# ezorita/seeq

Hardware: AMD Instinct MI355X
Metric: lines/s scanned (20 bp pattern, d=3, 150 bp reads; GB/s in gb_per_s) (higher is better)
Workload: dtype int (u16 automaton state ids; exact-pass columns u32 bit-vectors)

## Files before the change

seeq_amd/csrc/seeq_pair.h:

```cpp
#ifndef SEEQ_PAIR_H_
#define SEEQ_PAIR_H_

#define PAIR_X2(K) \
   asm("v_xor_b32_sdwa %0, %1, %2 dst_sel:DWORD dst_unused:UNUSED_PAD src0_sel:DWORD src1_sel:BYTE_" #K : "=v"(ada) : "v"(sa), "v"(ta)); \
   asm("v_xor_b32_sdwa %0, %1, %2 dst_sel:DWORD dst_unused:UNUSED_PAD src0_sel:DWORD src1_sel:BYTE_" #K : "=v"(adb) : "v"(sb), "v"(tb)); \
   sa = *(stream_lds_cu16 *)(uintptr_t)ada; sb = *(stream_lds_cu16 *)(uintptr_t)adb; \
   __builtin_amdgcn_sched_barrier(0);

__device__ __forceinline__ uint32_t pair_prep(uint32_t w)
{
   const uint32_t u = w & 0x06060606u;
   return u | (u << 10);
}

__device__ __forceinline__ void pair_chk(uint32_t w, uint32_t &bad, uint32_t &nm, bool first_of_two)
{
   const uint32_t idx = (w >> 1) & 0x07070707u;
   bad = __builtin_amdgcn_sad_u8(w, __builtin_amdgcn_perm(0x4EFF0AFFu, 0x47544341u, idx), bad);
   const uint32_t nf = __builtin_amdgcn_perm(0x00000100u, 0u, idx);
   nm = first_of_two ? __builtin_amdgcn_udot4(nf, 0x10204080u, nm << 8, false) : __builtin_amdgcn_udot4(nf, 0x01020408u, nm, false);
}

__device__ __forceinline__ void pair_warm4x2(uint32_t &sa, uint32_t wa, uint32_t &sb, uint32_t wb, uint32_t &seena, uint32_t &seenb)
{
   const uint32_t ta = pair_prep(wa), tb = pair_prep(wb);
   uint32_t ada, adb;
   PAIR_X2(1) asm("v_or_b32 %0, %0, %1" : "+v"(seena) : "v"(sa)); asm("v_or_b32 %0, %0, %1" : "+v"(seenb) : "v"(sb));
   PAIR_X2(3) asm("v_or_b32 %0, %0, %1" : "+v"(seena) : "v"(sa)); asm("v_or_b32 %0, %0, %1" : "+v"(seenb) : "v"(sb));
}

template <bool CHK>
__device__ __forceinline__ void pair_own4x2(uint32_t &sa, uint32_t wa, uint32_t &hma, uint32_t &nma, uint32_t &sb, uint32_t wb, uint32_t &hmb, uint32_t &nmb,
                                            uint32_t &bad, bool first_of_two)
{
   const uint32_t ta = pair_prep(wa), tb = pair_prep(wb);
   uint32_t ada, adb;
   PAIR_X2(1)
   asm volatile("" : "+v"(wa));
   if (CHK) pair_chk(wa, bad, nma, first_of_two);
   asm volatile("" : "+v"(bad), "+v"(nma));
   __builtin_amdgcn_sched_barrier(0);
   hma = __builtin_amdgcn_alignbit(sa, hma, 1); hmb = __builtin_amdgcn_alignbit(sb, hmb, 1);
   asm volatile("" : "+v"(hma), "+v"(hmb));
   PAIR_X2(3)
   asm volatile("" : "+v"(wb));
   if (CHK) pair_chk(wb, bad, nmb, first_of_two);
   asm volatile("" : "+v"(bad), "+v"(nmb));
   __builtin_amdgcn_sched_barrier(0);
   hma = __builtin_amdgcn_alignbit(sa, hma, 1); hmb = __builtin_amdgcn_alignbit(sb, hmb, 1);
   asm volatile("" : "+v"(hma), "+v"(hmb));
}

__device__ __forceinline__ uint32_t pair_word8(const fused_v4u &p, const fused_v4u &q, int k)
{
   return k == 0 ? p.x : k == 1 ? p.y : k == 2 ? p.z : k == 3 ? p.w : k == 4 ? q.x : k == 5 ? q.y : k == 6 ? q.z : q.w;
}

typedef uint32_t pair_u32_unaligned __attribute__((aligned(1)));

__device__ __forceinline__ uint32_t pair_nonbase_mask32(const fused_v4u &a, const fused_v4u &b)
{
   const uint32_t w[8] = {a.x, a.y, a.z, a.w, b.x, b.y, b.z, b.w};
   uint32_t h[2];
#pragma unroll
   for (int g = 0; g < 2; g++) {
      uint32_t acc = 0;
#pragma unroll
      for (int k = 4 * g; k < 4 * g + 4; k += 2) {
         uint32_t f[2];
#pragma unroll
         for (int u = 0; u < 2; u++) {
            const uint32_t x = w[k + u];
            const uint32_t t = x ^ __builtin_amdgcn_perm(0x474E5554u, 0x43FF41FFu, x & 0x07070707u);
            f[u] = (((t & 0x5F5F5F5Fu) + 0x7F7F7F7Fu) | t) & 0x80808080u;
         }
         acc = __builtin_amdgcn_udot4(f[0], 0x10204080u, __builtin_amdgcn_udot4(f[1], 0x01020408u, acc << 8, false), false);
      }
      h[g] = acc;
   }
   return (h[0] << 9) | (h[1] >> 7);
}

__device__ __forceinline__ uint32_t pair_count_before(const uint32_t (&m)[4], const uint32_t (&c)[5], uint32_t b)
{
   const uint32_t r = b >> 5, lz = b & 31u;
   const uint32_t mr = r == 0 ? m[0] : r == 1 ? m[1] : r == 2 ? m[2] : r == 3 ? m[3] : 0u;
   const uint32_t cr = r == 0 ? c[0] : r == 1 ? c[1] : r == 2 ? c[2] : r == 3 ? c[3] : c[4];
   return cr + (lz ? (uint32_t)__popc(mr >> (32u - lz)) : 0u);
}

template <int WU, bool CHK>
__device__ __forceinline__ void pair_walk(const fused_v4u (&v)[8], uint32_t halo, bool halo_nl, uint32_t (&hm)[2], uint32_t (&nmask)[4], uint32_t &tile_bad)
{
   constexpr int NQ = 8, NM = 4;
   uint32_t sa = 0, sb = 0, hma = 0, hmb = 0, seena = 0, seenb = 0, bad = 0, nma = 0, nmb = 0;
#pragma unroll
   for (int k = 8 - WU; k < 8; k++)
      pair_warm4x2(sa, stream_from_prev_lane(pair_word8(v[NQ - 2], v[NQ - 1], k), halo_nl ? 0x0A0A0A0Au : (uint32_t)__builtin_amdgcn_readlane((int)halo, k)),
                        sb, pair_word8(v[NQ / 2 - 2], v[NQ / 2 - 1], k), seena, seenb);
#pragma unroll
   for (int q = 0; q < NQ / 2; q++) {
      pair_own4x2<CHK>(sa, v[q].x, hma, nma, sb, v[q + NQ / 2].x, hmb, nmb, bad, true);
      pair_own4x2<CHK>(sa, v[q].y, hma, nma, sb, v[q + NQ / 2].y, hmb, nmb, bad, false);
      pair_own4x2<CHK>(sa, v[q].z, hma, nma, sb, v[q + NQ / 2].z, hmb, nmb, bad, true);
      pair_own4x2<CHK>(sa, v[q].w, hma, nma, sb, v[q + NQ / 2].w, hmb, nmb, bad, false);
      if (CHK && (q & 1)) { nmask[q >> 1] = nma; nmask[(q >> 1) + NM / 2] = nmb; nma = 0; nmb = 0; }
   }
   tile_bad = bad;
   hm[0] = __builtin_bitreverse32(hma) | ((seena & 1u) << 31);
   hm[1] = __builtin_bitreverse32(hmb) | ((seenb & 1u) << 31);
}

template <int WU, bool FA, bool IG = false, bool LL = false>
__global__ __launch_bounds__(64 * STREAM_NW, 8) void k_pair(FusedArgs a)
{
   static_assert(!(FA && IG), "SQ_IGNORE on FASTA input stays with k_stream");
   static_assert(!(LL && (FA || IG)), "the long-line variant serves plain text under SQ_FAIL / SQ_CONVERT");
   constexpr int NW = STREAM_NW;
   constexpr int CH = 128;
   constexpr int NQ = CH / 16;
   constexpr int NM = CH / 32;
   constexpr uint32_t TB = 64u * CH;
   static_assert(WU >= 4 && WU <= 8, "warm-up is 16 .. 32 bytes");
   extern __shared__ __align__(16) uint8_t dsmem[];
   const int tid = threadIdx.x, lane = tid & 63;
   const int wave = __builtin_amdgcn_readfirstlane(tid >> 6);
   {
      const fused_v4u *src = reinterpret_cast<const fused_v4u *>(a.dfa);
      for (uint32_t i = tid; i < a.dfa_rows; i += 64 * NW) reinterpret_cast<fused_v4u *>(dsmem)[i] = src[i];
   }
   __syncthreads();

   const uint32_t gwave = blockIdx.x * NW + wave, nwaves = gridDim.x * NW;
   if (a.clk_probe != nullptr && blockIdx.x == 0 && tid == 0) { a.clk_probe[0] = __builtin_readcyclecounter(); a.clk_probe[1] = wall_clock64(); }
   uint32_t wv_lines = 0, wv_hitlines = 0, wv_hdrs = 0, slice_pos = 0;
   bool wv_overflow = false;
   uint32_t wv_dirty = 0, wv_lastnl = 0;
   uint32_t dmode = 0;
   uint4 *slice = a.tmp + (size_t)gwave * a.slice_cap;
   const uint64_t lim = a.seg_base + a.seg_len;
   const uint64_t last = a.nbytes - 1;

   fused_v4u v[NQ];
   uint32_t halo = 0;
   uint32_t tile = gwave;
   while (tile < a.ntiles) {
      const uint64_t t0 = a.seg_base + (uint64_t)tile * TB;
      const bool partial = tile + 1 == a.ntiles && (a.seg_len % TB) != 0;
      const uint32_t next = tile + nwaves;
      uint32_t lane_off = (uint32_t)lane * CH;
      asm volatile("" : "+v"(lane_off));
      const uint64_t my = t0 + lane_off;
      {
         if (!partial) {
            const uint8_t *p = a.text + my;
#pragma unroll
            for (int q = 0; q < NQ; q++) v[q] = *reinterpret_cast<const fused_v4u_unaligned *>(p + 16 * q);
            uint32_t lid;
            asm volatile("v_mbcnt_lo_u32_b32 %0, -1, 0\n\tv_mbcnt_hi_u32_b32 %0, -1, %0" : "=v"(lid));
            halo = *reinterpret_cast<const pair_u32_unaligned *>(a.text + (t0 >= 32 ? t0 - 32 : 0) + ((lid & 7u) << 2));
         } else {
#pragma unroll
            for (int q = 0; q < NQ; q++) v[q] = dfa_load16(a.text, my + 16 * q, lim);
            const fused_v4u h0 = dfa_load16(a.text, t0 >= 32 ? t0 - 32 : 0, lim), h1 = dfa_load16(a.text, t0 >= 32 ? t0 - 16 : 0, lim);
            halo = pair_word8(h0, h1, 0);
#pragma unroll
            for (int k = 1; k < 8; k++) halo = (lane & 7) == k ? pair_word8(h0, h1, k) : halo;
         }
      }
      const bool halo_nl = t0 < 32;
      uint32_t hm[2], nmask[NM];
      if (!dmode) {
         uint32_t tile_bad;
         pair_walk<WU, true>(v, halo, halo_nl, hm, nmask, tile_bad);
         const uint64_t badlanes = __ballot(tile_bad != 0);
         dmode = (uint32_t)__builtin_amdgcn_readfirstlane(badlanes != 0 ? 1 : 0);
         if (LL && lane == 0) { a.tile_dirty[tile] = badlanes != 0 ? 1u : 0u; a.tile_dmask[tile] = badlanes; }
      } else {
         uint32_t unused;
         pair_walk<WU, false>(v, halo, halo_nl, hm, nmask, unused);
         if (LL && lane == 0) { a.tile_dirty[tile] = 1u; a.tile_dmask[tile] = ~0ull; }
      }
      if (dmode) {
         wv_dirty |= 1u;
#pragma unroll
         for (int r = 0; r < NM; r++) nmask[r] = stream_nl_mask32(v[2 * r], v[2 * r + 1], false);
      }
      uint32_t valid = CH;
      if (partial) {
         valid = lim > my ? (lim - my < CH ? (uint32_t)(lim - my) : (uint32_t)CH) : 0u;
#pragma unroll
         for (int r = 0; r < NM; r++) {
            const uint32_t lo = 32u * r;
            nmask[r] &= valid <= lo ? 0u : (valid >= lo + 32 ? 0xFFFFFFFFu : ~(0xFFFFFFFFu >> (valid - lo)));
         }
#pragma unroll
         for (int x = 0; x < 2; x++) {
            const uint32_t vx = valid <= 64u * x ? 0u : (valid - 64u * x >= 64u ? 64u : valid - 64u * x);
            const uint32_t np = (vx + 1u) >> 1;
            hm[x] &= np >= 32u ? 0xFFFFFFFFu : ~(0xFFFFFFFFu >> np);
         }
      }
      uint32_t mk[2] = {0u, 0u};
      const uint32_t walk_hm[2] = {hm[0], hm[1]};
      if (IG) {
         uint32_t e_tail = 0;
         if (t0 <= last && last < t0 + TB) { if (a.text[last] != '\n') e_tail = (uint32_t)(last - t0) + 1u; }
         else if (!partial && a.text[t0 + TB] == '\n') e_tail = TB;
         e_tail = (uint32_t)__builtin_amdgcn_readfirstlane((int)e_tail);
         uint32_t vm[NM], sk[NM], dn[NM];
#pragma unroll
         for (int r = 0; r < NM; r++) {
            const uint32_t lo = 32u * r;
            vm[r] = valid <= lo ? 0u : (valid >= lo + 32 ? 0xFFFFFFFFu : ~(0xFFFFFFFFu >> (valid - lo)));
            sk[r] = dmode ? pair_nonbase_mask32(v[2 * r], v[2 * r + 1]) & ~nmask[r] & vm[r] : 0u;
            dn[r] = ~(nmask[r] | sk[r]) & vm[r];
         }
         uint32_t cD[5], cS[5];
         cD[0] = 0; cS[0] = 0;
#pragma unroll
         for (int r = 0; r < NM; r++) { cD[r + 1] = cD[r] + (uint32_t)__popc(dn[r]); cS[r + 1] = cS[r] + (uint32_t)__popc(sk[r]); }
         const uint32_t end_after = (uint32_t)__builtin_amdgcn_update_dpp(0, (int)(nmask[0] >> 31), 0x130, 0xf, 0xf, true);
         uint32_t b_tail = 0;
         if (e_tail && (uint32_t)lane == (e_tail - 1u) / CH) b_tail = e_tail - (uint32_t)lane * CH;
         if (end_after) b_tail = CH;
         uint32_t baseD = 0, baseS = 0, seen_end = 0, firstP = 0, first_pq = 0;
         auto mark = [&](uint32_t pq) { if (pq < 32u) mk[0] |= 0x80000000u >> pq; else mk[1] |= 0x80000000u >> (pq - 32u); };
         auto line_end = [&](uint32_t b, uint32_t Dc, uint32_t Sc) {
            if (b >= 1u) {
               const uint32_t lineD = Dc + baseD, lineS = Sc + baseS;
               if (!seen_end) { firstP = 0x80000000u | (lineS << 14) | lineD; first_pq = (b - 1u) >> 1; }
               else if (lineS != 0u && lineD >= a.ig_thr) mark((b - 1u) >> 1);
            }
            baseD = 0u - Dc; baseS = 0u - Sc; seen_end = 1u;
         };
#pragma unroll
         for (int r = 0; r < NM; r++) {
            uint32_t mm = nmask[r];
            while (mm) {
               const uint32_t lz = (uint32_t)__builtin_clz(mm);
               mm &= ~(0x80000000u >> lz);
               line_end(32u * r + lz, cD[r] + (uint32_t)__popc((dn[r] >> 1) >> (31u - lz)), cS[r] + (uint32_t)__popc((sk[r] >> 1) >> (31u - lz)));
            }
         }
         if (__ballot(b_tail != 0u)) {
            if (b_tail == CH) line_end(CH, cD[4], cS[4]);
            else if (b_tail) line_end(b_tail, pair_count_before(dn, cD, b_tail), pair_count_before(sk, cS, b_tail));
         }
         uint32_t P = (seen_end << 31) | (cD[4] + baseD) | ((cS[4] + baseS) << 14);
#define PAIR_SEG(ctrl, rmask) { const uint32_t y = (uint32_t)__builtin_amdgcn_update_dpp(0, (int)P, ctrl, rmask, 0xf, true); P = (P >> 31) ? P : y + P; }
         PAIR_SEG(0x111, 0xf) PAIR_SEG(0x112, 0xf) PAIR_SEG(0x114, 0xf) PAIR_SEG(0x118, 0xf) PAIR_SEG(0x142, 0xa) PAIR_SEG(0x143, 0xc)
#undef PAIR_SEG
         const uint32_t starts_line = (uint32_t)__builtin_amdgcn_readfirstlane((t0 == 0 || (t0 >= 32 && ((uint32_t)__builtin_amdgcn_readlane((int)halo, 7) >> 24) == 0x0Au)) ? 1 : 0);
         const uint32_t before = stream_from_prev_lane(P, starts_line << 31);
         if ((firstP >> 31) && ((before >> 31) | starts_line)) {
            const uint32_t sum = (firstP & 0x0FFFFFFFu) + (before & 0x0FFFFFFFu);
            if ((sum >> 14) != 0u && (sum & 0x3FFFu) >= a.ig_thr) mark(first_pq);
         }
         {
            const uint32_t tile_valid = (uint32_t)__builtin_amdgcn_readfirstlane((int)(partial ? (uint32_t)(lim - t0) : TB));
            const uint32_t lv = (tile_valid - 1u) >> 7, bb = (tile_valid - 1u) & 127u;
            const uint32_t ng = (bb >> 5) == 0 ? nmask[0] : (bb >> 5) == 1 ? nmask[1] : (bb >> 5) == 2 ? nmask[2] : nmask[3];
            const uint32_t last_is_nl = (uint32_t)__builtin_amdgcn_readlane((int)((ng >> (31u - (bb & 31u))) & 1u), (int)lv);
            const bool buffer_last = t0 <= last && last < t0 + TB;
            if (!buffer_last && e_tail == 0u && !last_is_nl) {
               const uint32_t P63 = (uint32_t)__builtin_amdgcn_readlane((int)P, 63);
               const uint32_t started_here = (P63 >> 31) | starts_line;
               const uint64_t pk = t0 + tile_valid + 4u * (uint32_t)lane;
               uint32_t w = 0x0A0A0A0Au;
               if (pk + 4 <= a.nbytes) w = *reinterpret_cast<const pair_u32_unaligned *>(a.text + pk);
               else for (int i = 3; i >= 0; i--) w = (w << 8) | (pk + (uint64_t)i < a.nbytes ? (uint32_t)a.text[pk + i] : 0x0Au);
               const uint32_t nlf = nl_flags(w);
               const uint64_t nlb = __ballot(nlf != 0u);
               uint32_t qualifies = 1u;
               if (nlb != 0ull && started_here) {
                  const uint32_t F = (uint32_t)__builtin_ctzll(nlb);
                  const uint32_t nbytes_mine = (uint32_t)lane < F ? 4u : (uint32_t)lane == F ? ((uint32_t)__builtin_ctz(nlf) >> 3) : 0u;
                  const uint32_t keepm = nbytes_mine >= 4u ? 0xFFFFFFFFu : (1u << (8u * nbytes_mine)) - 1u;
                  const uint32_t y = (w ^ __builtin_amdgcn_perm(0x474E5554u, 0x43FF41FFu, w & 0x07070707u)) & keepm;
                  const uint32_t cs = (uint32_t)__popc((((y & 0x5F5F5F5Fu) + 0x7F7F7F7Fu) | y) & 0x80808080u);
                  const uint32_t tot = (uint32_t)__builtin_amdgcn_readlane((int)wave_incl_scan_u32((nbytes_mine - cs) | (cs << 16)), 63);
                  const uint32_t lineD = (P63 & 0x3FFFu) + (tot & 0xFFFFu), lineS = ((P63 >> 14) & 0x3FFFu) + (tot >> 16);
                  qualifies = (lineS != 0u && lineD >= a.ig_thr) ? 1u : 0u;
               }
               if (qualifies && (uint32_t)lane == lv) mark(bb >> 1);
            }
         }
         hm[0] |= mk[0]; hm[1] |= mk[1];
      }
      if (t0 <= last && last < t0 + TB) {
         const uint32_t o = (uint32_t)(last - t0);
         if ((uint32_t)lane == o / CH) {
            const uint32_t pos = o % CH;
#pragma unroll
            for (int r = 0; r < NM; r++)
               if ((pos >> 5) == (uint32_t)r) nmask[r] &= ~(0x80000000u >> (pos & 31));
         }
      }
      if (!LL && __ballot(((hm[0] & (hm[0] - 1u)) | (hm[1] & (hm[1] - 1u))) != 0)) {
#pragma unroll
         for (int x = 0; x < 2; x++) {
            const uint32_t n0 = nmask[2 * x], n1 = nmask[2 * x + 1], h = hm[x];
            const uint32_t f = n0 ? (uint32_t)__builtin_clz(n0) : (n1 ? 32u + (uint32_t)__builtin_clz(n1) : 64u);
            const uint32_t l = n1 ? 63u - (uint32_t)__builtin_ctz(n1) : (n0 ? 31u - (uint32_t)__builtin_ctz(n0) : 64u);
            const uint32_t na = f >= 64u ? 32u : (f + 1u) >> 1;
            const uint32_t sc = f >= 64u ? 32u : (l + 1u) >> 1;
            const uint32_t ma = na >= 32u ? 0xFFFFFFFFu : ~(0xFFFFFFFFu >> na);
            const uint32_t mc = sc >= 32u ? 0u : 0xFFFFFFFFu >> sc;
            const uint32_t ha = h & ma, hc = h & mc & ~ma;
            hm[x] = (h & ~ma & ~mc) | (ha ? (0x80000000u >> (uint32_t)__builtin_clz(ha)) | (ha & (0u - ha)) : 0u)
                                    | (hc ? (0x80000000u >> (uint32_t)__builtin_clz(hc)) | (hc & (0u - hc)) : 0u);
         }
      }
      uint32_t lane_nl = 0;
      const uint32_t lane_hits = (uint32_t)__popc(hm[0]) + (uint32_t)__popc(hm[1]);
#pragma unroll
      for (int r = 0; r < NM; r++) lane_nl += (uint32_t)__popc(nmask[r]);
      const uint32_t incl_h = wave_incl_scan_u32(lane_hits), incl_n = wave_incl_scan_u32(lane_nl);
      const uint32_t tot_h = (uint32_t)__builtin_amdgcn_readlane((int)incl_h, 63);
      const uint32_t tot_n = (uint32_t)__builtin_amdgcn_readlane((int)incl_n, 63);
      const uint32_t extra = (uint32_t)__builtin_amdgcn_readfirstlane((a.first_seg && tile == 0) ? 1 : 0);
      uint32_t dmask[NM], lane_hd = 0, excl_d = 0, tot_d = 0, hd_extra = 0;
#pragma unroll
      for (int r = 0; r < NM; r++) dmask[r] = 0;
      if (FA) {
#pragma unroll
         for (int r = 0; r < NM; r++) {
            uint32_t mm = nmask[r];
            while (mm) {
               const uint32_t lz = (uint32_t)__builtin_clz(mm);
               mm &= ~(0x80000000u >> lz);
               const uint64_t nxt = my + 32u * r + lz + 1;
               if (a.text[nxt] == '>') dmask[r] |= 0x80000000u >> lz;
            }
            lane_hd += (uint32_t)__popc(dmask[r]);
         }
         const uint32_t incl_d = wave_incl_scan_u32(lane_hd);
         excl_d = incl_d - lane_hd;
         tot_d = (uint32_t)__builtin_amdgcn_readlane((int)incl_d, 63);
         hd_extra = extra && a.text[0] == '>' ? 1u : 0u;
      }
      uint32_t incl_last = 0;
      if (tot_n && (tot_h || LL)) {
         uint32_t my_last = 0;
#pragma unroll
         for (int r = 0; r < NM; r++)
            if (nmask[r]) my_last = (uint32_t)lane * CH + 32u * r + (31u - (uint32_t)__builtin_ctz(nmask[r])) + 2u;
         incl_last = wave_incl_max_u32(my_last);
         if (LL) wv_lastnl = tile * TB + (uint32_t)__builtin_amdgcn_readlane((int)incl_last, 63) - 1u;
      }
      if (tot_h) {
         if (slice_pos + tot_h <= a.slice_cap) {
            uint32_t before = stream_from_prev_lane(incl_last, 0u);
            if (extra && before == 0) before = 1;
            if (lane_hits) {
               uint32_t ord = incl_h - lane_hits;
               uint32_t nlb = incl_n - lane_nl + extra - 1u - excl_d - hd_extra;
#pragma unroll
               for (int r = 0; r < NM; r++) {
                  uint32_t mm = (r & 1) ? hm[r >> 1] << 16 : hm[r >> 1] & 0xFFFF0000u;
                  const uint32_t mkm = (r & 1) ? mk[r >> 1] << 16 : mk[r >> 1] & 0xFFFF0000u;
                  const uint32_t wkm = (r & 1) ? walk_hm[r >> 1] << 16 : walk_hm[r >> 1] & 0xFFFF0000u;
                  while (mm) {
                     const uint32_t lp = (uint32_t)__builtin_clz(mm);
                     mm &= ~(0x80000000u >> lp);
                     const uint32_t isk = IG ? (((mkm << lp) >> 31) << 30) | ((((mkm & wkm) << lp) >> 31) << 29) : 0u;
                     uint32_t lz = 2u * lp + 1u;
                     if (partial && 32u * r + lz >= valid) lz = valid - 1u - 32u * r;
                     const uint32_t nlt = lz ? nmask[r] >> (32 - lz) : 0u;
                     const uint32_t nb = (uint32_t)__popc(nlt) - (FA && lz ? (uint32_t)__popc(dmask[r] >> (32 - lz)) : 0u);
                     const uint32_t st1 = nlt ? (uint32_t)lane * CH + 32u * r + lz - (uint32_t)__builtin_ctz(nlt) + 1u : before;
                     const uint32_t hp = (uint32_t)lane * CH + 32u * r + lz;
                     const uint32_t pos = st1 ? st1 - 1u : hp;
                     slice[slice_pos + ord] = make_uint4(tile | (st1 ? 0u : 0x80000000u) | isk, ord | ((hp - pos) << 13),
                                                         tile * TB + pos + a.pos_bias, nlb + nb);
                     ord++;
                  }
                  if (nmask[r]) before = (uint32_t)lane * CH + 32u * r + (31u - (uint32_t)__builtin_ctz(nmask[r])) + 2u;
                  nlb += (uint32_t)__popc(nmask[r]) - (uint32_t)__popc(dmask[r]);
               }
            }
            slice_pos += tot_h;
         } else {
            wv_overflow = true;
         }
      }
      if (lane == 0) {
         a.tile_cl[tile] = tot_n + extra - tot_d - hd_extra;
         a.tile_hits[tile] = tot_h;
      }
      if (!LL && tot_h && !tot_n && !partial && !(t0 <= last && last < t0 + TB)) wv_dirty |= 2u;
      wv_lines += tot_n + extra;
      wv_hdrs += tot_d + hd_extra;
      wv_hitlines += tot_h;
      tile = next;
   }
   if (lane == 0) {
      a.wg_hits[gwave] = wv_overflow ? 0u : slice_pos;
      a.wg_part[4 * gwave + 0] = wv_lines;
      a.wg_part[4 * gwave + 1] = wv_hdrs;
      if (LL) a.wg_lastnl[gwave] = wv_lastnl;
      a.wg_part[4 * gwave + 2] = wv_overflow ? (wv_hitlines | 0x80000000u) : wv_hitlines;
      a.wg_part[4 * gwave + 3] = wv_dirty;
   }   if (a.clk_probe != nullptr && blockIdx.x == 0 && tid == 0) { a.clk_probe[2] = __builtin_readcyclecounter(); a.clk_probe[3] = wall_clock64(); }
}

#undef PAIR_X2

#endif
```

Measured before the change: 26.70 billion.

## Pack newline/hit counts into one wave scan and replace max-scan with ballot+bpermute

Merges the two inclusive wave scans over newline and hit counts into a single scan of a packed 16-bit pair. The wave max-scan that located the previous newline is replaced by a ballot of lanes holding newlines plus one ds_bpermute from the nearest such lane, with last-newline positions found via ffbl. The per-hit emission loop now walks two 64-bit halves instead of four 32-bit quarters. The aim is fewer cross-lane scan steps per tile, at the cost of a 16-bit overflow assumption guarded by a static_assert and more intricate index arithmetic.

```diff
diff --git a/seeq_amd/csrc/seeq_pair.h b/seeq_amd/csrc/seeq_pair.h
--- a/seeq_amd/csrc/seeq_pair.h
+++ b/seeq_amd/csrc/seeq_pair.h
@@ -87,6 +87,19 @@
    const uint32_t mr = r == 0 ? m[0] : r == 1 ? m[1] : r == 2 ? m[2] : r == 3 ? m[3] : 0u;
    const uint32_t cr = r == 0 ? c[0] : r == 1 ? c[1] : r == 2 ? c[2] : r == 3 ? c[3] : c[4];
    return cr + (lz ? (uint32_t)__popc(mr >> (32u - lz)) : 0u);
+}
+
+__device__ __forceinline__ uint32_t pair_ffbl(uint32_t x)
+{
+   uint32_t r;
+   asm("v_ffbl_b32 %0, %1" : "=v"(r) : "v"(x));
+   return r;
+}
+
+__device__ __forceinline__ uint32_t pair_last_nl(const uint32_t (&m)[4])
+{
+   const uint32_t t01 = min(pair_ffbl(m[1]) | 64u, pair_ffbl(m[0]) | 96u), t23 = min(pair_ffbl(m[3]), pair_ffbl(m[2]) | 32u);
+   return 129u - min(t01, t23);
 }
 
 template <int WU, bool CHK>
@@ -316,9 +329,10 @@
       const uint32_t lane_hits = (uint32_t)__popc(hm[0]) + (uint32_t)__popc(hm[1]);
 #pragma unroll
       for (int r = 0; r < NM; r++) lane_nl += (uint32_t)__popc(nmask[r]);
-      const uint32_t incl_h = wave_incl_scan_u32(lane_hits), incl_n = wave_incl_scan_u32(lane_nl);
-      const uint32_t tot_h = (uint32_t)__builtin_amdgcn_readlane((int)incl_h, 63);
-      const uint32_t tot_n = (uint32_t)__builtin_amdgcn_readlane((int)incl_n, 63);
+      static_assert(64 * CH <= 0xFFFF, "a wave's newlines and candidates are counted in 16 bits each");
+      const uint32_t incl = wave_incl_scan_u32(lane_nl | (lane_hits << 16));
+      const uint32_t tot = (uint32_t)__builtin_amdgcn_readlane((int)incl, 63);
+      const uint32_t tot_n = tot & 0xFFFFu, tot_h = tot >> 16;
       const uint32_t extra = (uint32_t)__builtin_amdgcn_readfirstlane((a.first_seg && tile == 0) ? 1 : 0);
       uint32_t dmask[NM], lane_hd = 0, excl_d = 0, tot_d = 0, hd_extra = 0;
 #pragma unroll
@@ -340,44 +354,50 @@
          tot_d = (uint32_t)__builtin_amdgcn_readlane((int)incl_d, 63);
          hd_extra = extra && a.text[0] == '>' ? 1u : 0u;
       }
-      uint32_t incl_last = 0;
-      if (tot_n && (tot_h || LL)) {
-         uint32_t my_last = 0;
-#pragma unroll
-         for (int r = 0; r < NM; r++)
-            if (nmask[r]) my_last = (uint32_t)lane * CH + 32u * r + (31u - (uint32_t)__builtin_ctz(nmask[r])) + 2u;
-         incl_last = wave_incl_max_u32(my_last);
-         if (LL) wv_lastnl = tile * TB + (uint32_t)__builtin_amdgcn_readlane((int)incl_last, 63) - 1u;
+      const uint64_t nlm = __ballot(lane_nl != 0);
+      uint32_t lid;
+      asm volatile("v_mbcnt_lo_u32_b32 %0, -1, 0\n\tv_mbcnt_hi_u32_b32 %0, -1, %0" : "=v"(lid));
+      const uint32_t lbase = lid * CH;
+      uint32_t my_last = 0;
+      if (tot_h || (LL && tot_n)) {
+         my_last = lbase + pair_last_nl(nmask);
+         if (LL && tot_n) wv_lastnl = tile * TB + (uint32_t)__builtin_amdgcn_readlane((int)my_last, 63 - __builtin_clzll(nlm)) - 1u;
       }
       if (tot_h) {
          if (slice_pos + tot_h <= a.slice_cap) {
-            uint32_t before = stream_from_prev_lane(incl_last, 0u);
-            if (extra && before == 0) before = 1;
+            const uint64_t below = (nlm << (63u - lid)) & 0x7FFFFFFFFFFFFFFFull;
+            const uint32_t from = lid - (below ? (uint32_t)__builtin_clzll(below) : 0u);
+            uint32_t before = (uint32_t)__builtin_amdgcn_ds_bpermute((int)(from << 2), (int)my_last);
+            if (!below) before = extra;
             if (lane_hits) {
-               uint32_t ord = incl_h - lane_hits;
-               uint32_t nlb = incl_n - lane_nl + extra - 1u - excl_d - hd_extra;
-#pragma unroll
-               for (int r = 0; r < NM; r++) {
-                  uint32_t mm = (r & 1) ? hm[r >> 1] << 16 : hm[r >> 1] & 0xFFFF0000u;
-                  const uint32_t mkm = (r & 1) ? mk[r >> 1] << 16 : mk[r >> 1] & 0xFFFF0000u;
-                  const uint32_t wkm = (r & 1) ? walk_hm[r >> 1] << 16 : walk_hm[r >> 1] & 0xFFFF0000u;
+               uint32_t ord = (incl >> 16) - lane_hits;
+               uint32_t nlb = (incl & 0xFFFFu) - lane_nl + extra - 1u - excl_d - hd_extra;
+#pragma unroll
+               for (int x = 0; x < 2; x++) {
+                  uint32_t mm = hm[x];
+                  if (x == 1 && mm) {
+                     const uint32_t ta = min(pair_ffbl(nmask[1]), pair_ffbl(nmask[0]) | 32u);
+                     if (ta != 0xFFFFFFFFu) before = lbase + 65u - ta;
+                     nlb += (uint32_t)__popc(nmask[0]) + (uint32_t)__popc(nmask[1]) - (uint32_t)__popc(dmask[0]) - (uint32_t)__popc(dmask[1]);
+                  }
+                  const uint64_t nx = ((uint64_t)nmask[2 * x] << 32) | nmask[2 * x + 1], dx = ((uint64_t)dmask[2 * x] << 32) | dmask[2 * x + 1];
+                  const uint32_t mkm = mk[x], wkm = walk_hm[x];
                   while (mm) {
                      const uint32_t lp = (uint32_t)__builtin_clz(mm);
                      mm &= ~(0x80000000u >> lp);
                      const uint32_t isk = IG ? (((mkm << lp) >> 31) << 30) | ((((mkm & wkm) << lp) >> 31) << 29) : 0u;
-                     uint32_t lz = 2u * lp + 1u;
-                     if (partial && 32u * r + lz >= valid) lz = valid - 1u - 32u * r;
-                     const uint32_t nlt = lz ? nmask[r] >> (32 - lz) : 0u;
-                     const uint32_t nb = (uint32_t)__popc(nlt) - (FA && lz ? (uint32_t)__popc(dmask[r] >> (32 - lz)) : 0u);
-                     const uint32_t st1 = nlt ? (uint32_t)lane * CH + 32u * r + lz - (uint32_t)__builtin_ctz(nlt) + 1u : before;
-                     const uint32_t hp = (uint32_t)lane * CH + 32u * r + lz;
+                     uint32_t c = 64u * x + 2u * lp + 1u;
+                     if (partial && c >= valid) c = valid - 1u;
+                     const uint32_t sh = 64u * x + 63u - c;
+                     const uint64_t pre = (nx >> sh) & ~1ull;
+                     const uint32_t nb = (uint32_t)__popcll(pre) - (FA ? (uint32_t)__popcll((dx >> sh) & ~1ull) : 0u);
+                     const uint32_t hp = lbase + c;
+                     const uint32_t st1 = pre ? hp - (uint32_t)__builtin_ctzll(pre) + 2u : before;
                      const uint32_t pos = st1 ? st1 - 1u : hp;
                      slice[slice_pos + ord] = make_uint4(tile | (st1 ? 0u : 0x80000000u) | isk, ord | ((hp - pos) << 13),
                                                          tile * TB + pos + a.pos_bias, nlb + nb);
                      ord++;
                   }
-                  if (nmask[r]) before = (uint32_t)lane * CH + 32u * r + (31u - (uint32_t)__builtin_ctz(nmask[r])) + 2u;
-                  nlb += (uint32_t)__popc(nmask[r]) - (uint32_t)__popc(dmask[r]);
                }
             }
             slice_pos += tot_h;
@@ -390,9 +410,9 @@
          a.tile_hits[tile] = tot_h;
       }
       if (!LL && tot_h && !tot_n && !partial && !(t0 <= last && last < t0 + TB)) wv_dirty |= 2u;
-      wv_lines += tot_n + extra;
+      wv_lines = (uint32_t)__builtin_amdgcn_readfirstlane((int)(wv_lines + tot_n + extra));
       wv_hdrs += tot_d + hd_extra;
-      wv_hitlines += tot_h;
+      wv_hitlines = (uint32_t)__builtin_amdgcn_readfirstlane((int)(wv_hitlines + tot_h));
       tile = next;
    }
    if (lane == 0) {
```

After: 26.15 billion. 0.979x the previous value.
